# Z2PackDev/TBmodels

Measured on AMD Instinct MI355X. Metric: k-points/sec (H(k)+eig) at N_orb=64, N_R=4096, higher is better.
Workload: dtype f64; 1 GPU; cfg2: dense N_orb=64 N_R=4096, 100000 random k-points per GPU, eigenval (H(k)+eig); kpoints_per_gpu=100000, collective=none, rccl_ranks=0, eigensolver=auto

## Files before the change

### tbmodels_amd/csrc/tbk_api.hip

```cpp

#include <algorithm>
#include <cmath>
#include <cstdarg>
#include <cstdlib>
#include <cstring>
#include <dlfcn.h>
#include <functional>
#include <new>
#include <vector>

#include "tbk_internal.h"

static thread_local char g_err[1024] = "";

void tbk_set_error(const char* fmt, ...) {
    va_list ap;
    va_start(ap, fmt);
    vsnprintf(g_err, sizeof(g_err), fmt, ap);
    va_end(ap);
}

extern "C" const char* tbk_last_error(void) { return g_err; }
extern "C" const char* tbk_version(void) { return "tbk 0.1 (gfx950)"; }

// ... 68 lines not shown
            return;
        }
        tbk_range_push(kStageNames[stage]);
        (void)hipEventRecord(ev.start, stream);
    }
}

StageTimer::~StageTimer() {
    if (on) {
        (void)hipEventRecord(ev.stop, stream);
        tbk_range_pop();
        m->events.push_back(ev);
    }
}

static inline int64_t round_up(int64_t x, int64_t q) { return (x + q - 1) / q * q; }

static int require_device(int device) {
    int n = 0;
    if (hipGetDeviceCount(&n) != hipSuccess || n == 0) {
        (void)hipGetLastError();
        tbk_set_error("no HIP device visible: libtbk has no CPU path");
        return TBK_ERR_DEVICE;
    }
    if (device < 0 || device >= n) {
        tbk_set_error("device %d out of range (have %d)", device, n);
        return TBK_ERR_ARGUMENT;
    }
    TBK_HIP(hipSetDevice(device));
    return TBK_OK;
}

static int create_common(int device, int dim, int n_orb, int64_t n_r, const int32_t* R,
                         int64_t k_rows_per_r, tbk_model** out) {
    TBK_ARG(out != nullptr, "out is NULL");
    *out = nullptr;
    TBK_ARG(dim >= 1 && dim <= TBK_MAX_DIM, "dim must be in [1, 8]");
    TBK_ARG(n_orb >= 1 && n_orb <= 32768, "n_orb must be in [1, 32768]");
    TBK_ARG(n_r >= 0 && n_r < (int64_t(1) << 28), "n_r out of range");
    TBK_ARG(n_r == 0 || R != nullptr || k_rows_per_r == 1, "R is NULL");
    TBK_CHECK(require_device(device));

    tbk_model* m = new (std::nothrow) tbk_model();
    if (!m) {
        tbk_set_error("out of host memory");
        return TBK_ERR_MEMORY;
    }
    m->device = device;
    {
        int cus = 0;
        if (hipDeviceGetAttribute(&cus, hipDeviceAttributeMultiprocessorCount, device) == hipSuccess && cus > 0) m->n_cu = cus;
    }
    m->dim = dim;
    m->n_orb = n_orb;
    m->n_r = n_r;
    m->k2 = round_up(n_r * k_rows_per_r, TBK_BK);
    m->n_r_pad = m->k2 / k_rows_per_r;
    m->ncol = (int)((int64_t)n_orb * (n_orb + 1) / 2);
    m->ncol_pad = (int)round_up(m->ncol, TBK_BNP);

    int rc = TBK_OK;
    auto fail = [&](int code) {
        tbk_model_destroy(m);
        return code;
    };
#define TBK_TRY(expr)                           \
    do {                                        \
        rc = [&]() -> int {                     \
            expr;                               \
            return TBK_OK;                      \
        }();                                    \
        if (rc != TBK_OK) return fail(rc);      \
    } while (0)

    TBK_TRY(TBK_HIP(hipStreamCreateWithFlags(&m->stream, hipStreamNonBlocking)));
    TBK_TRY(TBK_HIP(hipStreamCreateWithFlags(&m->stream_eig, hipStreamNonBlocking)));
    TBK_TRY(TBK_HIP(hipStreamCreateWithFlags(&m->stream_ql, hipStreamNonBlocking)));
    for (int b = 0; b < 2; ++b) {
        TBK_TRY(TBK_HIP(hipEventCreateWithFlags(&m->ev_hk[b], hipEventDisableTiming)));
        TBK_TRY(TBK_HIP(hipEventCreateWithFlags(&m->ev_tri[b], hipEventDisableTiming)));
        TBK_TRY(TBK_HIP(hipEventCreateWithFlags(&m->ev_ql[b], hipEventDisableTiming)));
        TBK_TRY(TBK_HIP(hipEventCreateWithFlags(&m->ev_out[b], hipEventDisableTiming)));
        if (b == 0) TBK_TRY(TBK_HIP(hipEventCreateWithFlags(&m->ev_sync, hipEventDisableTiming | hipEventReleaseToSystem)));
    }
    TBK_TRY(TBK_ROCBLAS(rocblas_create_handle(&m->blas)));
    TBK_TRY(TBK_ROCBLAS(rocblas_set_stream(m->blas, m->stream)));
    TBK_TRY(TBK_CHECK(m->ws_flag.reserve(2 * sizeof(int))));
    TBK_TRY(TBK_HIP(hipMemsetAsync(m->ws_flag.ptr, 0, 2 * sizeof(int), m->stream)));
    m->h_stage_bytes = std::max<size_t>(size_t(320) << 10,
                                        n_orb <= 1024 ? (size_t)n_orb * n_orb * 16 + (size_t)n_orb * dim * 8 + (size_t(64) << 10) : 0);
    if (hipHostMalloc(&m->h_stage, m->h_stage_bytes, hipHostMallocNonCoherent) != hipSuccess) {
        (void)hipGetLastError();
        m->h_stage = nullptr;
        m->h_stage_bytes = 0;
    }

    {
        std::vector<int32_t> colmap((size_t)m->ncol_pad, -1);
        size_t e = 0;
        for (int i = 0; i < n_orb; ++i)
            for (int j = i; j < n_orb; ++j) colmap[e++] = (int32_t)((i << 16) | j);
        TBK_TRY(TBK_HIP(hipMalloc((void**)&m->d_colmap, colmap.size() * sizeof(int32_t))));
        TBK_TRY(TBK_HIP(hipMemcpy(m->d_colmap, colmap.data(), colmap.size() * sizeof(int32_t),
                                  hipMemcpyHostToDevice)));
        m->staged_bytes += (int64_t)(colmap.size() * sizeof(int32_t));
    }
    if (n_r > 0 && R != nullptr && k_rows_per_r == 2) m->h_R.assign(R, R + (size_t)n_r * dim);
    if (m->n_r_pad > 0 && R != nullptr) {
        std::vector<int32_t> r_pad((size_t)m->n_r_pad * dim, 0);
        std::memcpy(r_pad.data(), R, (size_t)n_r * dim * sizeof(int32_t));
        TBK_TRY(TBK_HIP(hipMalloc((void**)&m->d_R, r_pad.size() * sizeof(int32_t))));
        TBK_TRY(TBK_HIP(hipMemcpy(m->d_R, r_pad.data(), r_pad.size() * sizeof(int32_t),
                                  hipMemcpyHostToDevice)));
        m->staged_bytes += (int64_t)(r_pad.size() * sizeof(int32_t));
    }
#undef TBK_TRY
    *out = m;
    return TBK_OK;
}

extern "C" int tbk_model_create_dense(int device, int dim, int n_orb, int64_t n_r, const int32_t* R,
                                      const double* hop, tbk_model** out) {
    TBK_ARG(out != nullptr, "out is NULL");
    *out = nullptr;
    TBK_ARG(n_r == 0 || hop != nullptr, "hop is NULL");
    tbk_model* m = nullptr;
    TBK_CHECK(create_common(device, dim, n_orb, n_r, R, 2, &m));
    m->sparse = false;
    int rc = TBK_OK;
    double* d_raw = nullptr;
    const size_t raw_bytes = (size_t)n_r * n_orb * n_orb * 2 * sizeof(double);
    rc = [&]() -> int {
        if (raw_bytes) {
            TBK_HIP(hipMalloc((void**)&d_raw, raw_bytes));
            TBK_HIP(hipMemcpyAsync(d_raw, hop, raw_bytes, hipMemcpyHostToDevice, m->stream));
        }
        TBK_CHECK(tbk_stage_dense(m, d_raw));
        TBK_HIP(hipStreamSynchronize(m->stream));
        return TBK_OK;
    }();
    if (d_raw) (void)hipFree(d_raw);
    if (rc != TBK_OK) {
        tbk_model_destroy(m);
        return rc;
    }
    *out = m;
    return TBK_OK;
}

extern "C" int tbk_model_create_csr(int device, int dim, int n_orb, int64_t n_r, const int32_t* R,
                                    const int64_t* r_ptr, const int32_t* row, const int32_t* col,
                                    const double* val, tbk_model** out) {
    TBK_ARG(out != nullptr, "out is NULL");
    *out = nullptr;
    TBK_ARG(n_r >= 0, "n_r out of range");
    TBK_ARG(n_r == 0 || r_ptr != nullptr, "r_ptr is NULL");
    const int64_t nnz = n_r > 0 ? r_ptr[n_r] : 0;
    TBK_ARG(n_r == 0 || r_ptr[0] == 0, "r_ptr[0] must be 0");
    TBK_ARG(nnz >= 0, "negative nnz");
    TBK_ARG(nnz == 0 || (row && col && val), "row/col/val is NULL");
    for (int64_t r = 0; r < n_r; ++r) TBK_ARG(r_ptr[r] <= r_ptr[r + 1], "r_ptr not monotone");
    for (int64_t t = 0; t < nnz; ++t)
        TBK_ARG(row[t] >= 0 && row[t] < n_orb && col[t] >= 0 && col[t] < n_orb,
                "row/col index out of range");

    tbk_model* m = nullptr;
    TBK_CHECK(create_common(device, dim, n_orb, n_r, R, 2, &m));
    m->sparse = true;

    auto packed_index = [n_orb](int i, int j) -> int64_t {
        return (int64_t)i * n_orb - (int64_t)i * (i - 1) / 2 + (j - i);
    };
    std::vector<int64_t> cptr((size_t)m->ncol + 1, 0);
    for (int64_t t = 0; t < nnz; ++t) {
        const int i = std::min(row[t], col[t]), j = std::max(row[t], col[t]);
        cptr[(size_t)packed_index(i, j) + 1]++;
    }
    for (int e = 0; e < m->ncol; ++e) cptr[(size_t)e + 1] += cptr[(size_t)e];
    std::vector<int32_t> rec_r((size_t)nnz);
    std::vector<double> rec_v((size_t)nnz * 2);
    {
        std::vector<int64_t> cursor(cptr.begin(), cptr.end() - 1);
        for (int64_t r = 0; r < n_r; ++r)
            for (int64_t t = r_ptr[r]; t < r_ptr[r + 1]; ++t) {
                const int i = row[t], j = col[t];
                const int kind = (i == j) ? 2 : (i < j ? 0 : 1);
                const int64_t e = packed_index(std::min(i, j), std::max(i, j));
                const int64_t slot = cursor[(size_t)e]++;
                rec_r[(size_t)slot] = (int32_t)((kind << 28) | (int32_t)r);
                rec_v[(size_t)slot * 2] = val[2 * t];
                rec_v[(size_t)slot * 2 + 1] = val[2 * t + 1];
            }
    }
    m->nnz_rec = nnz;
    int rc = [&]() -> int {
        TBK_HIP(hipMalloc((void**)&m->d_cptr, cptr.size() * sizeof(int64_t)));
        TBK_HIP(hipMemcpy(m->d_cptr, cptr.data(), cptr.size() * sizeof(int64_t), hipMemcpyHostToDevice));
        m->staged_bytes += (int64_t)(cptr.size() * sizeof(int64_t));
        if (nnz > 0) {
            TBK_HIP(hipMalloc((void**)&m->d_rec_r, (size_t)nnz * sizeof(int32_t)));
// ... 744 lines not shown
        }
        const int rc_inline = eigenval_device_impl(m, m->ws_k.as<double>(), k, nk, m->ws_out.as<double>());
        m->h_k_inline = nullptr;
        TBK_CHECK(rc_inline);
        {
            const int64_t count = nk * m->n_orb;
            const unsigned blocks = (unsigned)std::min<int64_t>((count + 255) / 256, 64);
            hipLaunchKernelGGL(export_small_kernel, dim3(blocks), dim3(256), 0, m->stream, m->ws_out.as<double>(), count,
                               m->ws_flag.as<int>(), reinterpret_cast<double*>(st + e_off), flag);
            TBK_HIP(hipGetLastError());
        }
        TBK_CHECK(wait_main_stream(m));
        std::memcpy(E_out, st + e_off, e_bytes);
        if (flag[0] != 0 || flag[1] != 0) return tbk_eigenval_check(m);
        return TBK_OK;
    }
    TBK_HIP(hipMemcpyAsync(m->ws_k.ptr, k, k_bytes, hipMemcpyHostToDevice, m->stream));
    TBK_CHECK(eigenval_device_impl(m, m->ws_k.as<double>(), k, nk, m->ws_out.as<double>()));
    TBK_HIP(hipMemcpyAsync(E_out, m->ws_out.ptr, e_bytes, hipMemcpyDeviceToHost, m->stream));
    return tbk_eigenval_check(m);
}

extern "C" int tbk_tridiagonal_reduce(int device, int n_orb, int64_t nk, const double* H, int method, double* d, double* e,
                                      double* H_reduced) {
    TBK_ARG(nk >= 0, "nk < 0");
    TBK_ARG(n_orb >= 1 && (n_orb <= 64 || tbk_eig_stream_supported(n_orb)),
            "n_orb must be in [1, 4096] (larger matrices go through rocSOLVER as a whole)");
    TBK_ARG(method >= TBK_REDUCE_AUTO && method <= TBK_REDUCE_TWO_STAGE, "unknown reduction method");
    TBK_ARG(method != TBK_REDUCE_TWO_STAGE || tbk_eig_band_supported(n_orb), "the two-stage reduction handles 64 < n_orb <= 4096");
    TBK_ARG(method != TBK_REDUCE_ONE_STAGE || n_orb <= 512, "the one-stage reduction handles n_orb <= 512");
    if (nk == 0) return TBK_OK;
    TBK_ARG(H && d && e, "H / d / e is NULL");
    tbk_model* m = nullptr;
    TBK_CHECK(create_common(device, 1, n_orb, 0, nullptr, 2, &m));
    const size_t n = (size_t)n_orb, mat_bytes = n * n * 2 * sizeof(double);
    int rc = [&]() -> int {
        TBK_LOCK(m);
        m->call_nk = nk;
        TBK_CHECK(m->ws_H.reserve((size_t)nk * mat_bytes));
        TBK_CHECK(m->ws_E.reserve((size_t)nk * n * 2 * sizeof(double)));
        TBK_HIP(hipMemcpyAsync(m->ws_H.ptr, H, (size_t)nk * mat_bytes, hipMemcpyHostToDevice, m->stream));
        if (tbk_eig_small_supported(n_orb))
            TBK_CHECK(tbk_launch_tridiag(m, m->stream, m->ws_H.as<double>(), nk, m->ws_E.as<double>()));
        else
            TBK_CHECK(tbk_launch_tridiag_stream(m, m->stream, m->ws_H.as<double>(), nk, m->ws_E.as<double>(), method));
        TBK_HIP(hipMemcpyAsync(d, m->ws_E.ptr, (size_t)nk * n * sizeof(double), hipMemcpyDeviceToHost, m->stream));
        TBK_HIP(hipMemcpyAsync(e, m->ws_E.as<double>() + (size_t)nk * n, (size_t)nk * n * sizeof(double), hipMemcpyDeviceToHost,
                               m->stream));
        if (H_reduced)
            TBK_HIP(hipMemcpyAsync(H_reduced, m->ws_H.ptr, (size_t)nk * mat_bytes, hipMemcpyDeviceToHost, m->stream));
        TBK_HIP(hipStreamSynchronize(m->stream));
        return TBK_OK;
    }();
    tbk_model_destroy(m);
    return rc;
}

__global__ void __launch_bounds__(256) random_hermitian_kernel(double* __restrict__ H, int n, int64_t nk) {
    const int64_t total = nk * (int64_t)n * n;
    for (int64_t t = (int64_t)blockIdx.x * 256 + threadIdx.x; t < total; t += (int64_t)gridDim.x * 256) {
        const int64_t mat = t / ((int64_t)n * n);
        const int r = (int)((t / n) % n), c = (int)(t % n);
        const int i = r < c ? r : c, j = r < c ? c : r;
        uint64_t x = (uint64_t)mat * 0x9E3779B97F4A7C15ull + (uint64_t)i * 0xBF58476D1CE4E5B9ull + (uint64_t)j * 0x94D049BB133111EBull + 1;
        x ^= x >> 30; x *= 0xBF58476D1CE4E5B9ull; x ^= x >> 27; x *= 0x94D049BB133111EBull; x ^= x >> 31;
        const double re = (double)(int64_t)(x >> 11) * (1.0 / 9007199254740992.0) - 0.5;
        x ^= x >> 29; x *= 0x9E3779B97F4A7C15ull; x ^= x >> 32;
        const double im = (double)(int64_t)(x >> 11) * (1.0 / 9007199254740992.0) - 0.5;
        H[2 * t] = re;
        H[2 * t + 1] = i == j ? 0.0 : (r < c ? im : -im);
    }
}

extern "C" int tbk_reduce_standalone(int device, int n_orb, int64_t nk, int reps, double* us_per_matrix) {
    TBK_ARG(us_per_matrix != nullptr, "us_per_matrix is NULL");
    TBK_ARG(nk >= 1 && reps >= 1, "nk / reps < 1");
    TBK_ARG(n_orb >= 1 && (n_orb <= 64 || tbk_eig_stream_supported(n_orb)), "n_orb must be in [1, 4096]");
    for (int q = 0; q < 3; ++q) us_per_matrix[q] = 0.0;
    tbk_model* m = nullptr;
    TBK_CHECK(create_common(device, 1, n_orb, 0, nullptr, 2, &m));
    const size_t n = (size_t)n_orb, mat_bytes = n * n * 2 * sizeof(double);
    DevBuf pristine;
    hipEvent_t ev[2] = {nullptr, nullptr};
    int rc = [&]() -> int {
        TBK_LOCK(m);
        m->call_nk = nk;
        TBK_CHECK(pristine.reserve((size_t)nk * mat_bytes));
        TBK_CHECK(m->ws_H.reserve((size_t)nk * mat_bytes));
        TBK_CHECK(m->ws_E.reserve((size_t)nk * n * 2 * sizeof(double)));
        TBK_HIP(hipEventCreate(&ev[0]));
        TBK_HIP(hipEventCreate(&ev[1]));
        hipLaunchKernelGGL(random_hermitian_kernel, dim3(4096), dim3(256), 0, m->stream, pristine.as<double>(), n_orb, nk);
        TBK_HIP(hipGetLastError());
        const bool band = !tbk_eig_small_supported(n_orb) && tbk_eig_two_stage(m);
        if (band) {
            TBK_CHECK(m->ws_band.reserve((size_t)nk * tbk_band_scratch_per_matrix(n_orb)));
            TBK_CHECK(m->ws_bandmat[0].reserve((size_t)nk * tbk_band_bytes_per_matrix(n_orb)));
        }
        for (int what = 0; what < (band ? 3 : 1); ++what) {
            float sum = 0.0f;
            for (int r = 0; r <= reps; ++r) {
                if (what != 2)
                    TBK_HIP(hipMemcpyAsync(m->ws_H.ptr, pristine.ptr, (size_t)nk * mat_bytes, hipMemcpyDeviceToDevice, m->stream));
                TBK_HIP(hipEventRecord(ev[0], m->stream));
                if (what == 0) {
                    if (tbk_eig_small_supported(n_orb))
                        TBK_CHECK(tbk_launch_tridiag(m, m->stream, m->ws_H.as<double>(), nk, m->ws_E.as<double>()));
                    else
                        TBK_CHECK(tbk_launch_tridiag_stream(m, m->stream, m->ws_H.as<double>(), nk, m->ws_E.as<double>(), TBK_REDUCE_AUTO));
                } else if (what == 1) {
                    TBK_CHECK(tbk_launch_band_reduce(m, m->stream, m->ws_H.as<double>(), nk, m->ws_band.ptr, m->ws_bandmat[0].ptr));
                } else {
                    TBK_CHECK(tbk_launch_band_chase(m, m->stream, m->ws_bandmat[0].ptr, nk, m->ws_E.as<double>()));
                }
                TBK_HIP(hipEventRecord(ev[1], m->stream));
                TBK_HIP(hipEventSynchronize(ev[1]));
                float ms = 0.0f;
                TBK_HIP(hipEventElapsedTime(&ms, ev[0], ev[1]));
                if (r > 0) sum += ms;
            }
            us_per_matrix[what] = (double)sum / reps * 1e3 / (double)nk;
        }
        return TBK_OK;
    }();
    for (auto& e : ev)
        if (e) (void)hipEventDestroy(e);
    pristine.release();
    tbk_model_destroy(m);
    return rc;
}

extern "C" int tbk_kdotp_create(int device, int dim, int n_orb, int64_t n_p, const int32_t* powers,
                                const double* coeffs, tbk_kdotp** out) {
    TBK_ARG(out != nullptr, "out is NULL");
    *out = nullptr;
    TBK_ARG(n_p == 0 || (powers && coeffs), "powers / coeffs is NULL");
    for (int64_t t = 0; t < n_p * dim; ++t) TBK_ARG(powers[t] >= 0, "negative power");
    tbk_model* m = nullptr;
    TBK_CHECK(create_common(device, dim, n_orb, n_p, nullptr, 1, &m));
    m->kdotp = true;
    double* d_raw = nullptr;
    const size_t raw_bytes = (size_t)n_p * n_orb * n_orb * 2 * sizeof(double);
    int rc = [&]() -> int {
        if (n_p > 0) {
            TBK_HIP(hipMalloc((void**)&m->d_powers, (size_t)n_p * dim * sizeof(int32_t)));
            TBK_HIP(hipMemcpy(m->d_powers, powers, (size_t)n_p * dim * sizeof(int32_t), hipMemcpyHostToDevice));
            TBK_HIP(hipMalloc((void**)&d_raw, raw_bytes));
            TBK_HIP(hipMemcpyAsync(d_raw, coeffs, raw_bytes, hipMemcpyHostToDevice, m->stream));
        }
        TBK_CHECK(tbk_stage_kdotp(m, d_raw));
        TBK_HIP(hipStreamSynchronize(m->stream));
        return TBK_OK;
    }();
    if (d_raw) (void)hipFree(d_raw);
    if (rc != TBK_OK) {
        tbk_model_destroy(m);
        return rc;
    }
    tbk_kdotp* kp = new (std::nothrow) tbk_kdotp();
    if (!kp) {
        tbk_model_destroy(m);
        tbk_set_error("out of host memory");
        return TBK_ERR_MEMORY;
    }
    kp->core = m;
    *out = kp;
    return TBK_OK;
}

extern "C" void tbk_kdotp_destroy(tbk_kdotp* kp) {
    if (!kp) return;
    tbk_model_destroy(kp->core);
// ... 87 lines not shown
```

### tbmodels_amd/csrc/tbk_hk_dense.hip

```cpp

#include <algorithm>
#include <cstdlib>
#include <type_traits>

#include "tbk_internal.h"

namespace {

typedef double d4 __attribute__((ext_vector_type(4)));
typedef double d2 __attribute__((ext_vector_type(2)));
typedef __attribute__((address_space(1))) const void* gptr_t;
typedef __attribute__((address_space(3))) void* lptr_t;

constexpr int LDA = TBK_BM + 16;
constexpr int LDB = 2 * TBK_BNP + 16;
constexpr int STAGE_DOUBLES = TBK_BK * (LDA + LDB);

static_assert(TBK_BM == 128 && TBK_BNP == 64 && TBK_BK == 16, "wave decomposition is written for 128x64x16");

struct HkArgs {
    const double* A;
    const double* Bt;
    const int32_t* colmap;
    const double* kpts;
// ... 27 lines not shown
};

__device__ __forceinline__ double hk_kcomp(const HkArgs& a, int64_t kq, int d) { return a.k_inline ? a.k_val[d] : a.kpts[kq * a.dim + d]; }

template <int MODE, int CONV>
__device__ __forceinline__ void store_element(const HkArgs& a, int64_t kq, int oi, int oj, double re, double im) {
    if (CONV == 1 && oi != oj) {
        d2 ei, ej;
        if (a.k_inline) {
            double di = 0.0, dj = 0.0;
            for (int d = 0; d < a.dim; ++d) {
                di = fma(a.k_val[d], a.pos_raw[oi * a.dim + d], di);
                dj = fma(a.k_val[d], a.pos_raw[oj * a.dim + d], dj);
            }
            double sn, cs;
            sincospi(2.0 * di, &sn, &cs);
            ei = (d2){cs, sn};
            sincospi(2.0 * dj, &sn, &cs);
            ej = (d2){cs, sn};
        } else {
            ei = *reinterpret_cast<const d2*>(a.pos + ((size_t)kq * a.n_orb + oi) * 2);
            ej = *reinterpret_cast<const d2*>(a.pos + ((size_t)kq * a.n_orb + oj) * 2);
        }
        const double cs = ei[0] * ej[0] + ei[1] * ej[1], sn = ei[0] * ej[1] - ei[1] * ej[0];
        const double t = re * cs - im * sn;
        im = re * sn + im * cs;
        re = t;
    }
    double* hk = a.H + (size_t)kq * a.n_orb * a.n_orb * 2;
    *reinterpret_cast<d2*>(hk + ((size_t)oi * a.n_orb + oj) * 2) = (d2){re, im};
    if (MODE == HK_FULL && oi != oj) *reinterpret_cast<d2*>(hk + ((size_t)oj * a.n_orb + oi) * 2) = (d2){re, -im};
}

__device__ __forceinline__ bool tile_of_block(const HkArgs& a, int b, int& mt, int& nt) {
    if (a.xcd_rows == 0) {
        nt = b % a.nt_count;
        mt = b / a.nt_count;
        return mt < a.mt_count;
    }
    const int x = b & 7;
    const int t = b >> 3;
    const int base = a.mt_count >> 3, extra = a.mt_count & 7;
    const int rows = base + (x < extra ? 1 : 0);
    if (t >= rows * a.nt_count) return false;
    const int start = x * base + (x < extra ? x : extra);
    const int full = rows / a.xcd_rows;
    const int per_group = a.xcd_rows * a.nt_count;
    int row;
    if (t < full * per_group) {
        const int g = t / per_group, r = t % per_group;
        row = g * a.xcd_rows + r % a.xcd_rows;
        nt = r / a.xcd_rows;
    } else {
        const int tt = t - full * per_group, rr = rows - full * a.xcd_rows;
        row = full * a.xcd_rows + tt % rr;
        nt = tt / rr;
    }
    mt = start + row;
    return true;
}

template <int MODE, int CONV, bool SPLIT>
__global__ void __launch_bounds__(256, 2) hk_dense_kernel(const HkArgs a) {
    extern __shared__ __attribute__((aligned(16))) double smem[];

    const int unit = (int)blockIdx.x + a.block_offset;
// ... 97 lines not shown
    using ks2 = std::integral_constant<int, 2>;
    using ks3 = std::integral_constant<int, 3>;
    static_assert(TBK_BK == 16, "four K steps per stage are written out below");
    auto stage = [&](auto bufc, auto nextc, Frags& cur, bool more) {
        Frags f1 = read_frags(bufc, ks1{});
        mfma_step(cur);
        Frags f2 = read_frags(bufc, ks2{});
        mfma_step(f1);
        Frags f3 = read_frags(bufc, ks3{});
        mfma_step(f2);
        __syncthreads();
        if (more) cur = read_frags(nextc, ks0{});
        mfma_step(f3);
    };

    const int left = n_stage - s_begin;
    if (left > 0) issue_stage(buf0{});
    __syncthreads();
    Frags cur = read_frags(buf0{}, ks0{});
    for (int pair = 0; pair < (left >> 1); ++pair) {
        issue_stage(buf1{});
        stage(buf0{}, buf1{}, cur, true);
        const bool more = 2 * pair + 2 < left;
        if (more) issue_stage(buf0{});
        stage(buf1{}, buf0{}, cur, more);
    }
    if (left & 1) stage(buf0{}, buf1{}, cur, false);

#pragma unroll
    for (int j = 0; j < 2; ++j) {
        const int e = (int)n0 + (wn * 2 + j) * 16 + l15;
        const int32_t ij = a.colmap[e];
        if (ij < 0) continue;
        const int oi = ij >> 16, oj = ij & 0xffff;
#pragma unroll
        for (int i = 0; i < 4; ++i) {
#pragma unroll
            for (int r = 0; r < 4; ++r) {
                const int local = wm * 64 + i * 16 + l4 + 4 * r;
                const int64_t kq = m0 + local;
                if (local >= a.rows_per_tile || kq >= a.nk) continue;
                if (SPLIT) {
                    double* part =
                        a.p_tiles > 0
                            ? a.P2 + ((((size_t)blockIdx.y * a.p_tiles + blockIdx.x) * TBK_BM + local) * TBK_BNP +
                                      (wn * 2 + j) * 16 + l15) * 2
                            : a.P + (((size_t)split_y * a.p_rows + kq) * a.ncol_pad + e) * 2;
                    *reinterpret_cast<d2*>(part) = (d2){acc[i][j][0][r], acc[i][j][1][r]};
                } else {
                    store_element<MODE, CONV>(a, kq, oi, oj, acc[i][j][0][r], acc[i][j][1][r]);
                }
            }
        }
    }
}

constexpr int GEMV_U = 8;

template <int NKV, bool INLINE_PHASES>
__global__ void __launch_bounds__(256) hk_gemv_kernel(const HkArgs a, int strip_doubles) {
    extern __shared__ __attribute__((aligned(16))) double s_rows[];
    constexpr int U = NKV >= 32 ? 4 : GEMV_U;
    const int lane = threadIdx.x & 63;
    const int wave = __builtin_amdgcn_readfirstlane(threadIdx.x >> 6);
    const int nblk = a.ncol_pad >> 6;
    const int task = (int)blockIdx.x * 4 + wave;
    const int sl = task / nblk, cb = task - sl * nblk;
    if (sl >= a.splits) return;
    const int64_t n_pairs = a.k2 >> 1;
    const int64_t kk0 = 2 * (sl * n_pairs / a.splits);
    const int n_rows = (int)(2 * ((sl + 1) * n_pairs / a.splits) - kk0);
    const int64_t kbase = (int64_t)blockIdx.z * NKV;
    const int nk_here = (int)min((int64_t)NKV, a.nk - kbase);
    const int64_t ld2 = a.ncol_pad;
    const d2* rows = reinterpret_cast<const d2*>(a.Bt) + kk0 * ld2 + cb * 64;
    double* strip = s_rows + wave * strip_doubles;

    d2 buf0[U], buf1[U];
    double acc[NKV][2];
#pragma unroll
    for (int q = 0; q < NKV; ++q) acc[q][0] = acc[q][1] = 0.0;

    auto fetch = [&](d2 (&buf)[U], int base) {
#pragma unroll
        for (int u = 0; u < U; ++u) {
            const int r = min(base + u, n_rows - 1);
            buf[u] = __builtin_nontemporal_load(rows + (int64_t)r * ld2 + lane);
        }
    };
    auto consume = [&](const d2 (&buf)[U], int row) {
        const double* arow = INLINE_PHASES ? strip + row * NKV : a.A + (kk0 + row) * a.nk_pad + kbase;
        const int64_t lda = INLINE_PHASES ? NKV : a.nk_pad;
#pragma unroll
        for (int u = 0; u < U; ++u) {
            if (!INLINE_PHASES && row + u >= n_rows) break;
#pragma unroll
            for (int q = 0; q < NKV; ++q) {
                const double aq = arow[u * lda + q];
                acc[q][0] = fma(aq, buf[u][0], acc[q][0]);
// ... 76 lines not shown
    auto consume = [&](const d2 (&buf)[GEMV_U], int row) {
#pragma unroll
        for (int u = 0; u < GEMV_U; ++u) {
            const double aq = strip[row + u];
            acc0 = fma(aq, buf[u][0], acc0);
            acc1 = fma(aq, buf[u][1], acc1);
        }
    };
    for (int row = 0; row < n_rows; row += 2 * GEMV_U) {
        consume(buf0, row);
        __builtin_amdgcn_sched_barrier(0);
        fetch(buf0, row + 2 * GEMV_U);
        __builtin_amdgcn_sched_barrier(0);
        consume(buf1, row + GEMV_U);
        __builtin_amdgcn_sched_barrier(0);
        fetch(buf1, row + 3 * GEMV_U);
        __builtin_amdgcn_sched_barrier(0);
    }
    const bool hi = (lane & 8) != 0;
    const int el = (lane >> 4) * 16 + (lane & 7) * 2 + (hi ? 1 : 0);
    const double got = __shfl_xor(hi ? acc0 : acc1, 8, 64);
    part[wave * 64 + el] = hi ? (d2){got, acc1} : (d2){acc0, got};
    __syncthreads();
    if (wave != 0) return;
    const int e = cb * 64 + lane;
    const int32_t ij = a.colmap[e];
    if (ij < 0) return;
    d2 sum = part[lane];
#pragma unroll
    for (int w = 1; w < 4; ++w) {
        sum[0] += part[w * 64 + lane][0];
        sum[1] += part[w * 64 + lane][1];
    }
    store_element<MODE, CONV>(a, 0, ij >> 16, ij & 0xffff, sum[0], sum[1]);
}

template <int MODE, int CONV>
__global__ void __launch_bounds__(256) hk_finish_kernel(const HkArgs a) {
    const int64_t idx = (int64_t)blockIdx.x * 256 + threadIdx.x;
    const int e = (int)(idx % a.ncol_pad);
    const int64_t kq = idx / a.ncol_pad;
    if (kq >= a.nk) return;
    const int32_t ij = a.colmap[e];
    if (ij < 0) return;
    double re = 0.0, im = 0.0;
    for (int sp = 0; sp < a.splits; ++sp) {
        const d2 v = *reinterpret_cast<const d2*>(a.P + (((size_t)sp * a.p_rows + kq) * a.ncol_pad + e) * 2);
        re += v[0];
        im += v[1];
    }
    store_element<MODE, CONV>(a, kq, ij >> 16, ij & 0xffff, re, im);
}

template <int MODE, int CONV>
__global__ void __launch_bounds__(256) hk_finish_wide_kernel(const HkArgs a) {
    __shared__ double part[4][16][2];
    const int lane = threadIdx.x & 63, wave = threadIdx.x >> 6;
    const int el = lane & 15;
    const int j = wave * 4 + (lane >> 4);
    const int64_t idx = (int64_t)blockIdx.x * 16 + el;
    const int e = (int)(idx % a.ncol_pad);
    const int64_t kq = idx / a.ncol_pad;
    double re = 0.0, im = 0.0;
    if (kq < a.nk)
        for (int sp = j; sp < a.splits; sp += 16) {
            const d2 v = *reinterpret_cast<const d2*>(a.P + (((size_t)sp * a.p_rows + kq) * a.ncol_pad + e) * 2);
            re += v[0];
            im += v[1];
        }
    re += __shfl_xor(re, 16, 64);
    im += __shfl_xor(im, 16, 64);
    re += __shfl_xor(re, 32, 64);
    im += __shfl_xor(im, 32, 64);
    if (lane < 16) {
        part[wave][el][0] = re;
        part[wave][el][1] = im;
    }
    __syncthreads();
    if (threadIdx.x < 16 && kq < a.nk) {
        const int32_t ij = a.colmap[e];
        if (ij < 0) return;
        const double sr = (part[0][el][0] + part[1][el][0]) + (part[2][el][0] + part[3][el][0]);
        const double si = (part[0][el][1] + part[1][el][1]) + (part[2][el][1] + part[3][el][1]);
        store_element<MODE, CONV>(a, kq, ij >> 16, ij & 0xffff, sr, si);
    }
}

template <int MODE, int CONV>
__global__ void __launch_bounds__(256) hk_finish_tiles_kernel(const HkArgs a) {
    const int unit = (int)blockIdx.x + a.block_offset;
    const int split_y = unit / a.unit_grid;
    int mt_idx, nt_idx;
    if (!tile_of_block(a, unit - split_y * a.unit_grid, mt_idx, nt_idx)) return;
    const int el = threadIdx.x & (TBK_BNP - 1);
    const int e = nt_idx * TBK_BNP + el;
    const int32_t ij = a.colmap[e];
    if (ij < 0) return;
    for (int local = threadIdx.x / TBK_BNP; local < a.rows_per_tile; local += 256 / TBK_BNP) {
        const int64_t kq = (int64_t)mt_idx * a.rows_per_tile + local;
        if (kq >= a.nk) break;
        double re = 0.0, im = 0.0;
        for (int sp = 0; sp < a.sub_splits; ++sp) {
            const d2 v = *reinterpret_cast<const d2*>(
                a.P2 + ((((size_t)sp * a.p_tiles + blockIdx.x) * TBK_BM + local) * TBK_BNP + el) * 2);
            re += v[0];
            im += v[1];
        }
        if (a.splits > 1)
            *reinterpret_cast<d2*>(a.P + (((size_t)split_y * a.p_rows + kq) * a.ncol_pad + e) * 2) = (d2){re, im};
        else
            store_element<MODE, CONV>(a, kq, ij >> 16, ij & 0xffff, re, im);
    }
}

template <int MODE, int CONV>
hipError_t launch_gemv(tbk_model* m, const HkArgs& a, size_t lds, hipStream_t s) {
    const int tasks = (a.ncol_pad >> 6) * a.splits;
    const dim3 grid((unsigned)((tasks + 3) / 4), 1, (unsigned)((a.nk + 31) / 32));
    static std::atomic<bool> raised[2][6][TBK_MAX_DEVICES] = {};
#define TBK_GEMV(N, SLOT)                                                                                               \
    do {                                                                                                                \
        if (a.A == nullptr) {                                                                                           \
            hipError_t e1 = tbk_raise_lds_limit(reinterpret_cast<const void*>(&hk_gemv_kernel<N, true>), 160 * 1024, raised[0][SLOT]); \
            if (e1 != hipSuccess) return e1;                                                                            \
            hipLaunchKernelGGL((hk_gemv_kernel<N, true>), grid, dim3(256), lds, s, a, (int)(lds / 32));                                  \
        } else {                                                                                                        \
            hipError_t e1 = tbk_raise_lds_limit(reinterpret_cast<const void*>(&hk_gemv_kernel<N, false>), 160 * 1024, raised[1][SLOT]); \
            if (e1 != hipSuccess) return e1;                                                                            \
            hipLaunchKernelGGL((hk_gemv_kernel<N, false>), grid, dim3(256), lds, s, a, (int)(lds / 32));                                 \
        }                                                                                                               \
    } while (0)
    if (a.nk <= 1)
        TBK_GEMV(1, 0);
    else if (a.nk <= 2)
        TBK_GEMV(2, 1);
    else if (a.nk <= 4)
        TBK_GEMV(4, 2);
    else if (a.nk <= 8)
        TBK_GEMV(8, 3);
    else if (a.nk <= 16)
        TBK_GEMV(16, 4);
    else
        TBK_GEMV(32, 5);
#undef TBK_GEMV
// ... 277 lines not shown
```

### tbmodels_amd/csrc/tbk_internal.h

```cpp
#pragma once

#include <hip/hip_runtime.h>
#include <rocblas/rocblas.h>

#include <atomic>
#include <cstdlib>
#include <cstdint>
#include <cstdio>
#include <functional>
#include <mutex>
#include <string>
#include <vector>

#include "tbk.h"

constexpr int TBK_BM = 128;
constexpr int TBK_BNP = 64;
constexpr int TBK_BK = 16;
constexpr int TBK_CT = 16;
constexpr int TBK_MAX_DIM = 8;

void tbk_set_error(const char* fmt, ...);

#define TBK_HIP(expr)                                                                             \
    do {                                                                                          \
        hipError_t e_ = (expr);                                                                   \
        if (e_ != hipSuccess) {                                                                   \
            tbk_set_error("%s failed: %s (%s:%d)", #expr, hipGetErrorString(e_), __FILE__,        \
                          __LINE__);                                                              \
            return (e_ == hipErrorOutOfMemory) ? TBK_ERR_MEMORY : TBK_ERR_DEVICE;                 \
        }                                                                                         \
    } while (0)

#define TBK_ROCBLAS(expr)                                                                         \
    do {                                                                                          \
        rocblas_status s_ = (expr);                                                               \
        if (s_ != rocblas_status_success) {                                                       \
            tbk_set_error("%s failed: rocblas_status %d (%s:%d)", #expr, (int)s_, __FILE__,       \
                          __LINE__);                                                              \
            return (s_ == rocblas_status_memory_error) ? TBK_ERR_MEMORY : TBK_ERR_DEVICE;         \
        }                                                                                         \
    } while (0)

#define TBK_CHECK(expr)                                                                           \
    do {                                                                                          \
        int r_ = (expr);                                                                          \
        if (r_ != TBK_OK) return r_;                                                              \
    } while (0)

#define TBK_LOCK(m) std::lock_guard<std::recursive_mutex> tbk_lock_((m)->mu)

#define TBK_ARG(cond, msg)                                                                        \
    do {                                                                                          \
// ... 225 lines not shown
```

### tbmodels_amd/csrc/tbk_kdotp.hip

```cpp

#include <algorithm>

#include "tbk_internal.h"

namespace {

typedef double d2 __attribute__((ext_vector_type(2)));

__global__ void __launch_bounds__(256)
kdotp_phase_kernel(const double* __restrict__ k0, const int32_t* __restrict__ R, int dim, int64_t n_r,
                   double* __restrict__ ph) {
    const int64_t r = (int64_t)blockIdx.x * blockDim.x + threadIdx.x;
    if (r >= n_r) return;
    double dot = 0.0;
    for (int d = 0; d < dim; ++d) dot = fma(k0[d], (double)R[r * dim + d], dot);
    double s, c;
    sincospi(2.0 * dot, &s, &c);
    ph[2 * r] = c;
    ph[2 * r + 1] = s;
}

__global__ void __launch_bounds__(256)
kdotp_coeff_kernel(const double* __restrict__ Bt, const int32_t* __restrict__ colmap,
                   const int32_t* __restrict__ R, const double* __restrict__ ph,
                   const int32_t* __restrict__ powers, const double* __restrict__ prefactor, int dim,
                   int64_t n_r, int ncol, int ncol_pad, int n_orb, double* __restrict__ out) {
    const int e = blockIdx.x * blockDim.x + threadIdx.x;
    const int p = blockIdx.y;
    if (e >= ncol) return;
    const int32_t ij = colmap[e];
    const int oi = ij >> 16, oj = ij & 0xffff;
    int pw[TBK_MAX_DIM];
    int deg = 0;
    for (int d = 0; d < dim; ++d) {
        pw[d] = powers[p * dim + d];
        deg += pw[d];
    }
    const double sgn = (deg & 1) ? -1.0 : 1.0;
    const size_t tiles = ncol_pad / TBK_CT;
    const size_t col = ((size_t)(e / TBK_CT) * 2) * TBK_CT + e % TBK_CT;
    double xr = 0.0, xi = 0.0;
    for (int64_t r = 0; r < n_r; ++r) {
        double mono = 1.0;
        for (int d = 0; d < dim; ++d) {
            const double base = (double)R[r * dim + d];
            for (int t = 0; t < pw[d]; ++t) mono *= base;
        }
        if (mono == 0.0) continue;
        const double* row_c = Bt + (size_t)(2 * r) * tiles * 2 * TBK_CT + col;
        const double* row_s = Bt + (size_t)(2 * r + 1) * tiles * 2 * TBK_CT + col;
        const double s_re = row_c[0], d_im = row_c[TBK_CT], ms_im = row_s[0], d_re = row_s[TBK_CT];
        const double hr = 0.5 * (s_re + d_re), gr = 0.5 * (s_re - d_re);
        const double hi = 0.5 * (d_im - ms_im), gi = 0.5 * (-ms_im - d_im);
        const double c = ph[2 * r], s = ph[2 * r + 1];
        const double tr = (c * hr - s * hi) + sgn * (c * gr - s * gi);
        const double ti = (c * hi + s * hr) - sgn * (c * gi + s * gr);
        xr = fma(mono, tr, xr);
        xi = fma(mono, ti, xi);
    }
    const double fr = prefactor[2 * p], fi = prefactor[2 * p + 1];
    const double cr = fr * xr - fi * xi, ci = fr * xi + fi * xr;
    double* cp = out + (size_t)p * n_orb * n_orb * 2;
    *reinterpret_cast<d2*>(cp + ((size_t)oi * n_orb + oj) * 2) = (d2){cr, ci};
    if (oi != oj) *reinterpret_cast<d2*>(cp + ((size_t)oj * n_orb + oi) * 2) = (d2){cr, -ci};
}

}

extern "C" int tbk_kdotp_coefficients(tbk_model* m, const double* k0, int64_t n_p, const int32_t* powers,
                                      const double* prefactor, double* coeffs_out) {
    TBK_ARG(m != nullptr, "model is NULL");
    TBK_LOCK(m);
    TBK_ARG(!m->sparse && !m->kdotp, "construct_kdotp needs a dense tight-binding model handle");
    TBK_ARG(n_p >= 0 && n_p <= 65535, "n_p out of range");
    if (n_p == 0) return TBK_OK;
    TBK_ARG(k0 && powers && prefactor && coeffs_out, "NULL argument");
    for (int64_t t = 0; t < n_p * m->dim; ++t) TBK_ARG(powers[t] >= 0, "negative power");
    TBK_HIP(hipSetDevice(m->device));
    const size_t nn2 = (size_t)m->n_orb * m->n_orb * 2;
    const size_t out_bytes = (size_t)n_p * nn2 * sizeof(double);
    const size_t aux_bytes = (size_t)m->dim * sizeof(double) + (size_t)n_p * m->dim * sizeof(int32_t) +
                             (size_t)n_p * 2 * sizeof(double) + (size_t)std::max<int64_t>(m->n_r, 1) * 2 * sizeof(double);
    TBK_CHECK(m->ws_out.reserve(out_bytes));
    TBK_CHECK(m->ws_k.reserve(aux_bytes + 64));
    char* aux = m->ws_k.as<char>();
    double* d_k0 = reinterpret_cast<double*>(aux);
    double* d_pref = d_k0 + m->dim;
    double* d_ph = d_pref + n_p * 2;
    int32_t* d_pw = reinterpret_cast<int32_t*>(d_ph + std::max<int64_t>(m->n_r, 1) * 2);
    TBK_HIP(hipMemcpyAsync(d_k0, k0, m->dim * sizeof(double), hipMemcpyHostToDevice, m->stream));
    TBK_HIP(hipMemcpyAsync(d_pref, prefactor, (size_t)n_p * 2 * sizeof(double), hipMemcpyHostToDevice, m->stream));
    TBK_HIP(hipMemcpyAsync(d_pw, powers, (size_t)n_p * m->dim * sizeof(int32_t), hipMemcpyHostToDevice, m->stream));
    TBK_HIP(hipMemsetAsync(m->ws_out.ptr, 0, out_bytes, m->stream));
    if (m->n_r > 0) {
        hipLaunchKernelGGL(kdotp_phase_kernel, dim3((unsigned)((m->n_r + 255) / 256)), dim3(256), 0, m->stream, d_k0,
// ... 12 lines not shown
```

### tbmodels_amd/csrc/tbk_stage.hip

```cpp

#include "tbk_internal.h"

namespace {

__global__ void __launch_bounds__(256)
stage_dense_kernel(const double* __restrict__ hop, const int32_t* __restrict__ colmap, int n_orb,
                   int64_t n_r, int ncol_pad, double* __restrict__ Bt) {
    const int e = blockIdx.x * blockDim.x + threadIdx.x;
    const int64_t r = blockIdx.y;
    if (e >= ncol_pad || r >= n_r) return;
    const int32_t ij = colmap[e];
    if (ij < 0) return;
    const int i = ij >> 16, j = ij & 0xffff;
    const double* blk = hop + (size_t)r * n_orb * n_orb * 2;
    const double hr = blk[((size_t)i * n_orb + j) * 2], hi = blk[((size_t)i * n_orb + j) * 2 + 1];
    const double gr = blk[((size_t)j * n_orb + i) * 2], gi = blk[((size_t)j * n_orb + i) * 2 + 1];
    const size_t tiles = ncol_pad / TBK_CT;
    const size_t base0 = (((size_t)(2 * r) * tiles + e / TBK_CT) * 2) * TBK_CT + e % TBK_CT;
    const size_t base1 = (((size_t)(2 * r + 1) * tiles + e / TBK_CT) * 2) * TBK_CT + e % TBK_CT;
    Bt[base0] = hr + gr;
    Bt[base0 + TBK_CT] = hi - gi;
    Bt[base1] = -(hi + gi);
    Bt[base1 + TBK_CT] = hr - gr;
}

__global__ void __launch_bounds__(256)
stage_kdotp_kernel(const double* __restrict__ coeff, const int32_t* __restrict__ colmap, int n_orb,
                   int64_t n_p, int ncol_pad, double* __restrict__ Bt) {
    const int e = blockIdx.x * blockDim.x + threadIdx.x;
    const int64_t p = blockIdx.y;
    if (e >= ncol_pad || p >= n_p) return;
    const int32_t ij = colmap[e];
    if (ij < 0) return;
    const int i = ij >> 16, j = ij & 0xffff;
    const double* blk = coeff + (size_t)p * n_orb * n_orb * 2;
    const size_t tiles = ncol_pad / TBK_CT;
    const size_t base = (((size_t)p * tiles + e / TBK_CT) * 2) * TBK_CT + e % TBK_CT;
    Bt[base] = blk[((size_t)i * n_orb + j) * 2];
    Bt[base + TBK_CT] = blk[((size_t)i * n_orb + j) * 2 + 1];
}

}

int tbk_stage_dense(tbk_model* m, const double* d_hop_raw) {
    const size_t bytes = (size_t)m->k2 * m->ncol_pad * 2 * sizeof(double);
    if (bytes == 0) return TBK_OK;
    TBK_HIP(hipMalloc((void**)&m->d_B, bytes));
    m->staged_bytes += (int64_t)bytes;
    TBK_HIP(hipMemsetAsync(m->d_B, 0, bytes, m->stream));
    if (m->n_r > 0) {
        TBK_ARG(m->n_r <= 65535, "more than 65535 lattice vectors");
        dim3 grid((m->ncol_pad + 255) / 256, (unsigned)m->n_r);
// ... 23 lines not shown
```

Before: 961,400 k-points/s.

## Pack pairs of diagonal orbitals into one GEMM column slot and remap workgroups per XCD

For dense models, the diagonal entries of H(k) are real, so two diagonal orbitals now share one packed column slot. One uses the real half of the slot and the other uses the imaginary half. This cuts the GEMM column count from n(n+1)/2 to about n(n-1)/2 + n/2, reducing the cost of forming H(k). The staging, store and k·p paths all decode the new pair flag. A split-reduction kernel also remaps workgroup indices so that contiguous tasks land on the same XCD, aiming at better L2 locality. The risk is that the 15-bit column mask and the diagonal-pairing algebra must be exactly right for every path.

```diff
diff --git a/tbmodels_amd/csrc/tbk_api.hip b/tbmodels_amd/csrc/tbk_api.hip
--- a/tbmodels_amd/csrc/tbk_api.hip
+++ b/tbmodels_amd/csrc/tbk_api.hip
@@ -124,7 +124,7 @@
 }
 
 static int create_common(int device, int dim, int n_orb, int64_t n_r, const int32_t* R,
-                         int64_t k_rows_per_r, tbk_model** out) {
+                         int64_t k_rows_per_r, bool pair_diagonal, tbk_model** out) {
     TBK_ARG(out != nullptr, "out is NULL");
     *out = nullptr;
     TBK_ARG(dim >= 1 && dim <= TBK_MAX_DIM, "dim must be in [1, 8]");
@@ -148,7 +148,7 @@
     m->n_r = n_r;
     m->k2 = round_up(n_r * k_rows_per_r, TBK_BK);
     m->n_r_pad = m->k2 / k_rows_per_r;
-    m->ncol = (int)((int64_t)n_orb * (n_orb + 1) / 2);
+    m->ncol = (int)(pair_diagonal ? (int64_t)n_orb * (n_orb - 1) / 2 + (n_orb + 1) / 2 : (int64_t)n_orb * (n_orb + 1) / 2);
     m->ncol_pad = (int)round_up(m->ncol, TBK_BNP);
 
     int rc = TBK_OK;
@@ -190,8 +190,13 @@
     {
         std::vector<int32_t> colmap((size_t)m->ncol_pad, -1);
         size_t e = 0;
-        for (int i = 0; i < n_orb; ++i)
-            for (int j = i; j < n_orb; ++j) colmap[e++] = (int32_t)((i << 16) | j);
+        for (int i = 0; i < n_orb; ++i) {
+            if (!pair_diagonal)
+                colmap[e++] = (int32_t)((i << 16) | i);
+            else if (i % 2 == 0)
+                colmap[e++] = i + 1 < n_orb ? (int32_t)((i << 16) | TBK_SLOT_PAIR | (i + 1)) : (int32_t)((i << 16) | i);
+            for (int j = i + 1; j < n_orb; ++j) colmap[e++] = (int32_t)((i << 16) | j);
+        }
         TBK_TRY(TBK_HIP(hipMalloc((void**)&m->d_colmap, colmap.size() * sizeof(int32_t))));
         TBK_TRY(TBK_HIP(hipMemcpy(m->d_colmap, colmap.data(), colmap.size() * sizeof(int32_t),
                                   hipMemcpyHostToDevice)));
@@ -217,7 +222,7 @@
     *out = nullptr;
     TBK_ARG(n_r == 0 || hop != nullptr, "hop is NULL");
     tbk_model* m = nullptr;
-    TBK_CHECK(create_common(device, dim, n_orb, n_r, R, 2, &m));
+    TBK_CHECK(create_common(device, dim, n_orb, n_r, R, 2, true, &m));
     m->sparse = false;
     int rc = TBK_OK;
     double* d_raw = nullptr;
@@ -257,7 +262,7 @@
                 "row/col index out of range");
 
     tbk_model* m = nullptr;
-    TBK_CHECK(create_common(device, dim, n_orb, n_r, R, 2, &m));
+    TBK_CHECK(create_common(device, dim, n_orb, n_r, R, 2, false, &m));
     m->sparse = true;
 
     auto packed_index = [n_orb](int i, int j) -> int64_t {
@@ -1068,7 +1073,7 @@
     if (nk == 0) return TBK_OK;
     TBK_ARG(H && d && e, "H / d / e is NULL");
     tbk_model* m = nullptr;
-    TBK_CHECK(create_common(device, 1, n_orb, 0, nullptr, 2, &m));
+    TBK_CHECK(create_common(device, 1, n_orb, 0, nullptr, 2, false, &m));
     const size_t n = (size_t)n_orb, mat_bytes = n * n * 2 * sizeof(double);
     int rc = [&]() -> int {
         TBK_LOCK(m);
@@ -1114,7 +1119,7 @@
     TBK_ARG(n_orb >= 1 && (n_orb <= 64 || tbk_eig_stream_supported(n_orb)), "n_orb must be in [1, 4096]");
     for (int q = 0; q < 3; ++q) us_per_matrix[q] = 0.0;
     tbk_model* m = nullptr;
-    TBK_CHECK(create_common(device, 1, n_orb, 0, nullptr, 2, &m));
+    TBK_CHECK(create_common(device, 1, n_orb, 0, nullptr, 2, false, &m));
     const size_t n = (size_t)n_orb, mat_bytes = n * n * 2 * sizeof(double);
     DevBuf pristine;
     hipEvent_t ev[2] = {nullptr, nullptr};
@@ -1173,7 +1178,7 @@
     TBK_ARG(n_p == 0 || (powers && coeffs), "powers / coeffs is NULL");
     for (int64_t t = 0; t < n_p * dim; ++t) TBK_ARG(powers[t] >= 0, "negative power");
     tbk_model* m = nullptr;
-    TBK_CHECK(create_common(device, dim, n_orb, n_p, nullptr, 1, &m));
+    TBK_CHECK(create_common(device, dim, n_orb, n_p, nullptr, 1, false, &m));
     m->kdotp = true;
     double* d_raw = nullptr;
     const size_t raw_bytes = (size_t)n_p * n_orb * n_orb * 2 * sizeof(double);
diff --git a/tbmodels_amd/csrc/tbk_hk_dense.hip b/tbmodels_amd/csrc/tbk_hk_dense.hip
--- a/tbmodels_amd/csrc/tbk_hk_dense.hip
+++ b/tbmodels_amd/csrc/tbk_hk_dense.hip
@@ -83,6 +83,18 @@
     if (MODE == HK_FULL && oi != oj) *reinterpret_cast<d2*>(hk + ((size_t)oj * a.n_orb + oi) * 2) = (d2){re, -im};
 }
 
+template <int MODE, int CONV>
+__device__ __forceinline__ void store_slot(const HkArgs& a, int64_t kq, int32_t slot, double v0, double v1) {
+    const int oi = slot >> 16, oj = slot & 0x7fff;
+    if (slot & TBK_SLOT_PAIR) {
+        double* hk = a.H + (size_t)kq * a.n_orb * a.n_orb * 2;
+        *reinterpret_cast<d2*>(hk + ((size_t)oi * a.n_orb + oi) * 2) = (d2){v0, 0.0};
+        *reinterpret_cast<d2*>(hk + ((size_t)oj * a.n_orb + oj) * 2) = (d2){v1, 0.0};
+        return;
+    }
+    store_element<MODE, CONV>(a, kq, oi, oj, v0, v1);
+}
+
 __device__ __forceinline__ bool tile_of_block(const HkArgs& a, int b, int& mt, int& nt) {
     if (a.xcd_rows == 0) {
         nt = b % a.nt_count;
@@ -246,7 +258,6 @@
         const int e = (int)n0 + (wn * 2 + j) * 16 + l15;
         const int32_t ij = a.colmap[e];
         if (ij < 0) continue;
-        const int oi = ij >> 16, oj = ij & 0xffff;
 #pragma unroll
         for (int i = 0; i < 4; ++i) {
 #pragma unroll
@@ -262,7 +273,7 @@
                             : a.P + (((size_t)split_y * a.p_rows + kq) * a.ncol_pad + e) * 2;
                     *reinterpret_cast<d2*>(part) = (d2){acc[i][j][0][r], acc[i][j][1][r]};
                 } else {
-                    store_element<MODE, CONV>(a, kq, oi, oj, acc[i][j][0][r], acc[i][j][1][r]);
+                    store_slot<MODE, CONV>(a, kq, ij, acc[i][j][0][r], acc[i][j][1][r]);
                 }
             }
         }
@@ -278,7 +289,10 @@
     const int lane = threadIdx.x & 63;
     const int wave = __builtin_amdgcn_readfirstlane(threadIdx.x >> 6);
     const int nblk = a.ncol_pad >> 6;
-    const int task = (int)blockIdx.x * 4 + wave;
+    const int b = (int)blockIdx.x, n_wg = (int)gridDim.x;
+    const int xcd = b & 7, per_xcd = n_wg >> 3, extra = n_wg & 7;
+    const int wg = xcd * per_xcd + min(xcd, extra) + (b >> 3);
+    const int task = wg * 4 + wave;
     const int sl = task / nblk, cb = task - sl * nblk;
     if (sl >= a.splits) return;
     const int64_t n_pairs = a.k2 >> 1;
@@ -421,7 +435,7 @@
         sum[0] += part[w * 64 + lane][0];
         sum[1] += part[w * 64 + lane][1];
     }
-    store_element<MODE, CONV>(a, 0, ij >> 16, ij & 0xffff, sum[0], sum[1]);
+    store_slot<MODE, CONV>(a, 0, ij, sum[0], sum[1]);
 }
 
 template <int MODE, int CONV>
@@ -438,7 +452,7 @@
         re += v[0];
         im += v[1];
     }
-    store_element<MODE, CONV>(a, kq, ij >> 16, ij & 0xffff, re, im);
+    store_slot<MODE, CONV>(a, kq, ij, re, im);
 }
 
 template <int MODE, int CONV>
@@ -471,7 +485,7 @@
         if (ij < 0) return;
         const double sr = (part[0][el][0] + part[1][el][0]) + (part[2][el][0] + part[3][el][0]);
         const double si = (part[0][el][1] + part[1][el][1]) + (part[2][el][1] + part[3][el][1]);
-        store_element<MODE, CONV>(a, kq, ij >> 16, ij & 0xffff, sr, si);
+        store_slot<MODE, CONV>(a, kq, ij, sr, si);
     }
 }
 
@@ -498,7 +512,7 @@
         if (a.splits > 1)
             *reinterpret_cast<d2*>(a.P + (((size_t)split_y * a.p_rows + kq) * a.ncol_pad + e) * 2) = (d2){re, im};
         else
-            store_element<MODE, CONV>(a, kq, ij >> 16, ij & 0xffff, re, im);
+            store_slot<MODE, CONV>(a, kq, ij, re, im);
     }
 }
 
diff --git a/tbmodels_amd/csrc/tbk_internal.h b/tbmodels_amd/csrc/tbk_internal.h
--- a/tbmodels_amd/csrc/tbk_internal.h
+++ b/tbmodels_amd/csrc/tbk_internal.h
@@ -19,6 +19,8 @@
 constexpr int TBK_BK = 16;
 constexpr int TBK_CT = 16;
 constexpr int TBK_MAX_DIM = 8;
+
+constexpr int32_t TBK_SLOT_PAIR = 0x8000;
 
 void tbk_set_error(const char* fmt, ...);
 
diff --git a/tbmodels_amd/csrc/tbk_kdotp.hip b/tbmodels_amd/csrc/tbk_kdotp.hip
--- a/tbmodels_amd/csrc/tbk_kdotp.hip
+++ b/tbmodels_amd/csrc/tbk_kdotp.hip
@@ -29,7 +29,8 @@
     const int p = blockIdx.y;
     if (e >= ncol) return;
     const int32_t ij = colmap[e];
-    const int oi = ij >> 16, oj = ij & 0xffff;
+    const int oi = ij >> 16, oj = ij & 0x7fff;
+    const bool pair = (ij & TBK_SLOT_PAIR) != 0;
     int pw[TBK_MAX_DIM];
     int deg = 0;
     for (int d = 0; d < dim; ++d) {
@@ -39,7 +40,7 @@
     const double sgn = (deg & 1) ? -1.0 : 1.0;
     const size_t tiles = ncol_pad / TBK_CT;
     const size_t col = ((size_t)(e / TBK_CT) * 2) * TBK_CT + e % TBK_CT;
-    double xr = 0.0, xi = 0.0;
+    double xr = 0.0, xi = 0.0, yr = 0.0, yi = 0.0;
     for (int64_t r = 0; r < n_r; ++r) {
         double mono = 1.0;
         for (int d = 0; d < dim; ++d) {
@@ -49,18 +50,30 @@
         if (mono == 0.0) continue;
         const double* row_c = Bt + (size_t)(2 * r) * tiles * 2 * TBK_CT + col;
         const double* row_s = Bt + (size_t)(2 * r + 1) * tiles * 2 * TBK_CT + col;
-        const double s_re = row_c[0], d_im = row_c[TBK_CT], ms_im = row_s[0], d_re = row_s[TBK_CT];
-        const double hr = 0.5 * (s_re + d_re), gr = 0.5 * (s_re - d_re);
-        const double hi = 0.5 * (d_im - ms_im), gi = 0.5 * (-ms_im - d_im);
         const double c = ph[2 * r], s = ph[2 * r + 1];
-        const double tr = (c * hr - s * hi) + sgn * (c * gr - s * gi);
-        const double ti = (c * hi + s * hr) - sgn * (c * gi + s * gr);
-        xr = fma(mono, tr, xr);
-        xi = fma(mono, ti, xi);
+        auto term = [&](double s_re, double d_im, double ms_im, double d_re, double& ar, double& ai) {
+            const double hr = 0.5 * (s_re + d_re), gr = 0.5 * (s_re - d_re);
+            const double hi = 0.5 * (d_im - ms_im), gi = 0.5 * (-ms_im - d_im);
+            const double tr = (c * hr - s * hi) + sgn * (c * gr - s * gi);
+            const double ti = (c * hi + s * hr) - sgn * (c * gi + s * gr);
+            ar = fma(mono, tr, ar);
+            ai = fma(mono, ti, ai);
+        };
+        if (pair) {
+            term(row_c[0], 0.0, row_s[0], 0.0, xr, xi);
+            term(row_c[TBK_CT], 0.0, row_s[TBK_CT], 0.0, yr, yi);
+        } else {
+            term(row_c[0], row_c[TBK_CT], row_s[0], row_s[TBK_CT], xr, xi);
+        }
     }
     const double fr = prefactor[2 * p], fi = prefactor[2 * p + 1];
+    double* cp = out + (size_t)p * n_orb * n_orb * 2;
     const double cr = fr * xr - fi * xi, ci = fr * xi + fi * xr;
-    double* cp = out + (size_t)p * n_orb * n_orb * 2;
+    if (pair) {
+        *reinterpret_cast<d2*>(cp + ((size_t)oi * n_orb + oi) * 2) = (d2){cr, ci};
+        *reinterpret_cast<d2*>(cp + ((size_t)oj * n_orb + oj) * 2) = (d2){fr * yr - fi * yi, fr * yi + fi * yr};
+        return;
+    }
     *reinterpret_cast<d2*>(cp + ((size_t)oi * n_orb + oj) * 2) = (d2){cr, ci};
     if (oi != oj) *reinterpret_cast<d2*>(cp + ((size_t)oj * n_orb + oi) * 2) = (d2){cr, -ci};
 }
diff --git a/tbmodels_amd/csrc/tbk_stage.hip b/tbmodels_amd/csrc/tbk_stage.hip
--- a/tbmodels_amd/csrc/tbk_stage.hip
+++ b/tbmodels_amd/csrc/tbk_stage.hip
@@ -11,13 +11,22 @@
     if (e >= ncol_pad || r >= n_r) return;
     const int32_t ij = colmap[e];
     if (ij < 0) return;
-    const int i = ij >> 16, j = ij & 0xffff;
+    const int i = ij >> 16, j = ij & 0x7fff;
     const double* blk = hop + (size_t)r * n_orb * n_orb * 2;
-    const double hr = blk[((size_t)i * n_orb + j) * 2], hi = blk[((size_t)i * n_orb + j) * 2 + 1];
-    const double gr = blk[((size_t)j * n_orb + i) * 2], gi = blk[((size_t)j * n_orb + i) * 2 + 1];
     const size_t tiles = ncol_pad / TBK_CT;
     const size_t base0 = (((size_t)(2 * r) * tiles + e / TBK_CT) * 2) * TBK_CT + e % TBK_CT;
     const size_t base1 = (((size_t)(2 * r + 1) * tiles + e / TBK_CT) * 2) * TBK_CT + e % TBK_CT;
+    if (ij & TBK_SLOT_PAIR) {
+        const double hr = blk[((size_t)i * n_orb + i) * 2], hi = blk[((size_t)i * n_orb + i) * 2 + 1];
+        const double gr = blk[((size_t)j * n_orb + j) * 2], gi = blk[((size_t)j * n_orb + j) * 2 + 1];
+        Bt[base0] = hr + hr;
+        Bt[base0 + TBK_CT] = gr + gr;
+        Bt[base1] = -(hi + hi);
+        Bt[base1 + TBK_CT] = -(gi + gi);
+        return;
+    }
+    const double hr = blk[((size_t)i * n_orb + j) * 2], hi = blk[((size_t)i * n_orb + j) * 2 + 1];
+    const double gr = blk[((size_t)j * n_orb + i) * 2], gi = blk[((size_t)j * n_orb + i) * 2 + 1];
     Bt[base0] = hr + gr;
     Bt[base0 + TBK_CT] = hi - gi;
     Bt[base1] = -(hi + gi);
```

New measurement: 989,900 k-points/s (median of 6 runs). 3.0% higher.
